# meteofrance/py4cast

Measured on AMD Instinct MI355X. Metric: AR-training samples/sec (512x512x60 grid, 3-step rollout), higher is better.
Workload: dtype bf16; 1 GPU; HalfUNet scaled_ar rollout T=3, grid 512x512x60 (+5 forcings, 4 statics), WeightedLoss(MSE), AdamW, B=2/GPU; global_batch=2, parallelism=dp1, border_size=0, setup_steps=2, accumulate_grad_batches=1, hip_graph=False, deterministic_library_solvers=False, full=False

## Files before the change

### py4cast_amd/csrc/conv_bf16.hip

```cpp
#include <stdlib.h>

#include <type_traits>

#include "kernels.hpp"

namespace p4c {

typedef float f32x16 __attribute__((ext_vector_type(16)));
typedef float f32x4 __attribute__((ext_vector_type(4)));
typedef __bf16 bf16x8 __attribute__((ext_vector_type(8)));
typedef __bf16 bf16x4 __attribute__((ext_vector_type(4)));
typedef short s16x4 __attribute__((ext_vector_type(4)));

constexpr int BTW = 32;

#ifndef P4C_PRIO
#define P4C_PRIO 0
#endif
#ifndef P4C_EXP
#define P4C_EXP 0
#endif

#ifdef P4C_STAMPS
__device__ unsigned long long* g_stamps = nullptr;
// ... 1966 lines not shown
                           in_scale, in_shift, in_relu, out, out_cs, stat_partial, B, H, W);
    if (tag) prof_end(tag, stream);
    P4C_CHECK_LAUNCH("conv_fwd_bf16");
    return P4C_OK;
}

template <typename T, int CI, int KS>
static int launch_conv_wgrad_bf16(const T* in, const float* in_scale, const float* in_shift, int in_relu, const T* dout,
                                  float* partial, int G, int B, int H, int W, int in_cs, int ci_off, int part_cip,
                                  hipStream_t stream) {
    constexpr int HALO = KS / 2;
    constexpr int LH = 8 + 2 * HALO, LW = BTW + 2 * HALO;
    constexpr int ROWA = (CI * 2) % 256 == 64 ? CI * 2 : CI * 2 + 64;
    const size_t smem = (size_t)LH * LW * ROWA + (size_t)8 * BTW * 192;
    auto kern = conv_wgrad_bf16_kernel<T, CI, KS>;
    P4C_TRY(ensure_dyn_smem((const void*)kern, (int)smem));
    const int tag = (CI == 64 && KS == 3 && in_cs == 64) ? P4C_PROF_WGRAD3X3_C64 : 0;
    if (tag) prof_begin(tag, (int64_t)B * H * W, stream);
    hipLaunchKernelGGL(kern, dim3(G), dim3(256), smem, stream, in, in_scale, in_shift, in_relu, dout, partial, B, H, W,
                       in_cs, ci_off, part_cip);
    if (tag) prof_end(tag, stream);
    P4C_CHECK_LAUNCH("conv_wgrad_bf16");
    return P4C_OK;
}

int conv_bf16_stat_slots(int CI, int storage, int B, int H, int W, int ks) {
    if (CI > 96 && ks == 3) return conv_wide_stat_slots(H, W);
    if (conv_bf16_is_rows(storage, CI, ks, 1, 64, B, H, W)) return conv_rows_stat_slots(B, H, W);
    const int tiles = ((H + 3) / 4) * ((W + BTW - 1) / BTW);
    if (CI > 64 && storage != P4C_BF16) return tiles;
    int64_t ntiles = (int64_t)tiles * B;
    const int G = ntiles < num_cus() ? (int)ntiles : num_cus();
    return G * 4;
}

template <typename T>
static int conv_fwd_bf16_t(const T* in, int CI, const void* wp, int ks, const float* in_scale, const float* in_shift,
                           int in_relu, T* out, int out_cs, float* stat_partial, int B, int H, int W, int m_blocks,
                           hipStream_t stream) {
    const __bf16* w = (const __bf16*)wp;
    if (CI > 96 && ks == 3)
        return launch_conv_fwd_bf16_wide<T>(in, CI, w, in_scale, in_shift, in_relu, out, out_cs, stat_partial, B, H, W, m_blocks, stream);
#define P4C_CASE(ci, k, nb)                                                                                          \
    if (CI == ci && ks == k)                                                                                         \
        return launch_conv_fwd_bf16<T, ci, k, nb>(in, w, in_scale, in_shift, in_relu, out, out_cs, stat_partial, B, H, \
                                                  W, m_blocks, stream);
    P4C_CASE(32, 3, 2) P4C_CASE(64, 3, 2) P4C_CASE(96, 3, 1) P4C_CASE(32, 1, 2) P4C_CASE(64, 1, 2) P4C_CASE(96, 1, 1)
#undef P4C_CASE
    return fail(P4C_ERR_UNSUPPORTED, "conv_fwd_bf16: unsupported (CI=%d, ks=%d)", CI, ks);
}

static bool is_tile_ring(int storage, int CI, int ks, int m_blocks, int out_cs, int B, int H, int W) {
    return storage == P4C_BF16 && CI == 64 && ks == 3 && m_blocks == 1 && out_cs % 8 == 0 && B <= ring::MAXB &&
           (int64_t)H * W * out_cs * 2 < (int64_t)1 << 31;
}

bool conv_bf16_is_ring(int storage, int CI, int ks, int m_blocks, int out_cs, int B, int H, int W) {
    return conv_bf16_is_rows(storage, CI, ks, m_blocks, out_cs, B, H, W) || is_tile_ring(storage, CI, ks, m_blocks, out_cs, B, H, W);
}

bool conv_bf16_bwd_stats_ok(int storage, int B, int H, int W) {
    if (conv_bf16_is_rows(storage, 64, 3, 1, 64, B, H, W)) return conv_rows_stat_slots(B, H, W) <= NORM_BWD_MAX_BLOCKS;
    return is_tile_ring(storage, 64, 3, 1, 64, B, H, W) && B <= RING_BWD_STATS_MAXB && 4 * num_cus() <= NORM_BWD_MAX_BLOCKS;
}

int conv_fwd_bf16(const void* in, int storage, int CI, const void* wp, int ks, const float* in_scale,
                  const float* in_shift, int in_relu, void* out, int out_cs, float* stat_partial, int B, int H, int W,
                  int m_blocks, hipStream_t stream, const BatchFin* fin, const RingBwdStats* bst, int* nblk_out, const NormBwdCoef* nb) {
    if (conv_bf16_is_rows(storage, CI, ks, m_blocks, out_cs, B, H, W))
        return launch_conv3x3_bf16_rows(in, wp, ks, in_scale, in_shift, in_relu, out, out_cs, stat_partial, B, H, W, stream, fin, bst,
                                        nblk_out, nb);
    if (nb) return fail(P4C_ERR_INVALID, "conv_fwd_bf16: NormBwdCoef needs the row kernel");
    if (is_tile_ring(storage, CI, ks, m_blocks, out_cs, B, H, W))
        return launch_conv3x3_bf16_ring((const __bf16*)in, (const __bf16*)wp, in_scale, in_shift, in_relu, (__bf16*)out, out_cs,
                                        stat_partial, B, H, W, stream, fin, bst, nblk_out);
    if (fin || bst) return fail(P4C_ERR_INVALID, "conv_fwd_bf16: in-kernel statistics need the ring kernel");
    if (storage == P4C_BF16)
        return conv_fwd_bf16_t<__bf16>((const __bf16*)in, CI, wp, ks, in_scale, in_shift, in_relu, (__bf16*)out, out_cs,
                                       stat_partial, B, H, W, m_blocks, stream);
    return conv_fwd_bf16_t<float>((const float*)in, CI, wp, ks, in_scale, in_shift, in_relu, (float*)out, out_cs, stat_partial,
                                  B, H, W, m_blocks, stream);
}

int wgrad_reduce(const float* partial, int nslots, int ks, int CI_pad, int ci_lo, int ci_hi, int CO, int CI, float* grad,
                 hipStream_t stream);

template <typename T>
static int conv_wgrad_bf16_t(const T* in, int CI, int ks, const float* in_scale, const float* in_shift, int in_relu,
                             const T* dout, float* partial, int G, int B, int H, int W, int CO, int CIreal, float* grad,
                             hipStream_t stream, const NormBwdCoef* nb) {
    if (diag_skip(32)) return P4C_OK;
    if (CI % 32 != 0 || CI <= 0 || CI > 256) return fail(P4C_ERR_UNSUPPORTED, "conv_wgrad_bf16: unsupported CI=%d", CI);
    if (ks != 1 && ks != 3) return fail(P4C_ERR_UNSUPPORTED, "conv_wgrad_bf16: unsupported ks=%d", ks);
    const int tiles = ((H + 7) / 8) * ((W + BTW - 1) / BTW) * B;
    if (tiles < G) G = tiles;
    for (int off = 0; off < CI;) {
        const int chunk = (CI - off >= 64) ? 64 : 32;
        int rc;
        if (std::is_same<T, __bf16>::value && conv_wgrad_rows_ok(P4C_BF16, CI, off, 64, ks, G, B, H, W)) {
            int nslots = 0;
            if (off < CIreal) {
                P4C_TRY(launch_conv3x3_wgrad_bf16_rows(in, in_scale, in_shift, in_relu, dout, partial, G, B, H, W, stream, nb, &nslots, CI, off,
                                                       CIreal, CI));
                if (!diag_skip(8)) P4C_TRY(wgrad_reduce(partial, nslots, 3, CI, off, off + chunk, CO, CIreal, grad, stream));
            }
            off += chunk;
            continue;
        }
        const bool rem_ws = chunk == 32 && ks == 3 && off > 0 && diag_env("P4C_WGWS_REM") != nullptr;
        const bool ws_ok = (chunk == 64 || rem_ws) && (ks == 3 || diag_env("P4C_NO_WGWS_1X1") == nullptr) && std::is_same<T, __bf16>::value &&
                           B <= wgws::MAXB && diag_env("P4C_NO_WGWS") == nullptr;
        if (nb && !ws_ok) return fail(P4C_ERR_INVALID, "conv_wgrad_bf16: NormBwdCoef needs the role-split 3x3 kernel (64-channel chunk, bf16)");
        if (ws_ok)
            rc = launch_conv3x3_wgrad_bf16_ws((const __bf16*)in, in_scale, in_shift, in_relu, (const __bf16*)dout, partial, G, B, H, W,
                                              CI, off, CI, stream, nb, ks);
        else if (chunk == 64 && ks == 3)
            rc = launch_conv_wgrad_bf16<T, 64, 3>(in, in_scale, in_shift, in_relu, dout, partial, G, B, H, W, CI, off, CI, stream);
        else if (chunk == 32 && ks == 3)
            rc = launch_conv_wgrad_bf16<T, 32, 3>(in, in_scale, in_shift, in_relu, dout, partial, G, B, H, W, CI, off, CI, stream);
        else if (chunk == 64)
            rc = launch_conv_wgrad_bf16<T, 64, 1>(in, in_scale, in_shift, in_relu, dout, partial, G, B, H, W, CI, off, CI, stream);
        else
            rc = launch_conv_wgrad_bf16<T, 32, 1>(in, in_scale, in_shift, in_relu, dout, partial, G, B, H, W, CI, off, CI, stream);
        if (rc != P4C_OK) return rc;
        rc = diag_skip(8) ? P4C_OK : wgrad_reduce(partial, G * ((chunk == 64 || ws_ok) ? 1 : 2), ks, CI, off, off + chunk, CO, CIreal, grad, stream);
        if (rc != P4C_OK) return rc;
        off += chunk;
    }
    return P4C_OK;
}

bool conv_wgrad_bf16_takes_nb(int storage, int CI, int ks, int B) {
    if (storage != P4C_BF16 || ks != 3 || B > wgws::MAXB || diag_env("P4C_NO_WGWS")) return false;
    return CI % 64 == 0 || (CI % 64 == 32 && CI > 64 && diag_env("P4C_WGWS_REM") != nullptr);
}

int conv_wgrad_bf16(const void* in, int storage, int CI, int ks, const float* in_scale, const float* in_shift, int in_relu,
                    const void* dout, float* partial, int G, int B, int H, int W, int CO, int CIreal, float* grad,
                    hipStream_t stream, const NormBwdCoef* nb) {
    if (storage == P4C_BF16)
        return conv_wgrad_bf16_t<__bf16>((const __bf16*)in, CI, ks, in_scale, in_shift, in_relu, (const __bf16*)dout, partial, G,
                                         B, H, W, CO, CIreal, grad, stream, nb);
    if (nb) return fail(P4C_ERR_INVALID, "conv_wgrad_bf16: NormBwdCoef needs bf16 storage");
    return conv_wgrad_bf16_t<float>((const float*)in, CI, ks, in_scale, in_shift, in_relu, (const float*)dout, partial, G, B, H,
                                    W, CO, CIreal, grad, stream, nullptr);
}

int conv_wgrad_bf16_compact(const void* in, int in_cs, int ks, const void* dout, int dout_cs, float* partial, int G, int B, int H, int W,
                            int CO, int CIreal, float* grad, hipStream_t stream) {
    if (in_cs <= 0 || dout_cs <= 0 || in_cs > 64 || dout_cs > 64 || in_cs % 8 || dout_cs % 8 || (ks != 1 && ks != 3) || B > wgws::MAXB)
        return fail(P4C_ERR_UNSUPPORTED, "conv_wgrad_bf16_compact: unsupported shape (%d / %d channels, ks %d, B %d)", in_cs, dout_cs, ks, B);
    P4C_TRY(launch_conv3x3_wgrad_bf16_ws((const __bf16*)in, nullptr, nullptr, 0, (const __bf16*)dout, partial, G, B, H, W, in_cs, 0, 64, stream,
                                         nullptr, ks, dout_cs));
    const int tiles = ((H + 3) / 4) * ((W + BTW - 1) / BTW) * B;
    return wgrad_reduce(partial, tiles < G ? tiles : G, ks, 64, 0, 64, CO, CIreal, grad, stream);
}

#ifdef P4C_STAMPS
}
extern "C" int p4c_debug_set_stamps(void* p) {
    return hipMemcpyToSymbol(HIP_SYMBOL(p4c::g_stamps), &p, sizeof(p)) == hipSuccess ? 0 : -1;
}
namespace p4c {
#endif

int prep_weights_bf16(const float* w, int CO, int CI, int ks, int transpose_flip, int M_pad, int K_pad, void* out,
                      hipStream_t stream) {
    const int total = M_pad * K_pad * ks * ks;
    hipLaunchKernelGGL(prep_weights_bf16_kernel, dim3((total + 255) / 256), dim3(256), 0, stream, w, CO, CI, ks * ks,
                       transpose_flip, M_pad, K_pad, (__bf16*)out);
    P4C_CHECK_LAUNCH("prep_weights_bf16");
    return P4C_OK;
}

__global__ void __launch_bounds__(256) prep_weights_batch_kernel(PrepBatch pb) {
    if (blockIdx.x == 0 && blockIdx.y == 0 && (int)threadIdx.x < pb.n_zero) pb.zero_words[threadIdx.x] = 0u;
    const PrepJob& jb = pb.job[blockIdx.y];
    const int total = jb.M_pad * jb.K_pad * jb.ntaps;
    const int kv = pb.bf16 ? 8 : 4;
    const int ksteps = jb.K_pad / (2 * kv);
    for (int i = blockIdx.x * 256 + threadIdx.x; i < total; i += gridDim.x * 256) {
// ... 35 lines not shown
```

### py4cast_amd/csrc/conv_f32.hip

```cpp
#include "kernels.hpp"

namespace p4c {

typedef float f32x16 __attribute__((ext_vector_type(16)));
typedef float f32x4 __attribute__((ext_vector_type(4)));

constexpr int TW = 32;

__global__ void prep_weights_kernel(const float* __restrict__ w, int CO, int CI, int ntaps, int transpose_flip,
                                    int M_pad, int K_pad, float* __restrict__ out) {
    const int total = M_pad * K_pad * ntaps;
    for (int i = blockIdx.x * blockDim.x + threadIdx.x; i < total; i += gridDim.x * blockDim.x) {
        int t = i;
        const int s = t & 3; t >>= 2;
        const int m_l = t & 63; t >>= 6;
        const int h = t & 1; t >>= 1;
        const int q = t % (K_pad / 8); t /= (K_pad / 8);
        const int tap = t % ntaps;
        const int mb = t / ntaps;
        const int k = 8 * q + 4 * h + s, m = 64 * mb + m_l;
        float v = 0.0f;
        if (!transpose_flip) {
            if (m < CO && k < CI) v = w[((int64_t)m * CI + k) * ntaps + tap];
        } else {
// ... 185 lines not shown
    constexpr int KSPLIT = 4 / UNITS;
    constexpr int KSTEPS = TH * TW / 2 / KSPLIT;
    extern __shared__ __attribute__((aligned(16))) float lds[];
    float* lin = lds;
    float* ldo = lds + LH * LW * CIS;

    const int lane = threadIdx.x & 63, wv = threadIdx.x >> 6;
    const int r = lane & 31, h = lane >> 5;
    const int unit = wv % UNITS, ksl = wv / UNITS;
    const int cit = unit >> 1, cot = unit & 1;
    const int tiles_x = (W + TW - 1) / TW, tiles_y = (H + TH - 1) / TH;
    const int ntiles = tiles_x * tiles_y * B;
    const float* inb = in + ci_off;
    const float* scb = in_scale ? in_scale + ci_off : nullptr;
    const float* shb = in_shift ? in_shift + ci_off : nullptr;

    f32x16 acc[NTAPS];
#pragma unroll
    for (int t = 0; t < NTAPS; ++t)
#pragma unroll
        for (int i = 0; i < 16; ++i) acc[t][i] = 0.f;

    TileRegs<CI, LH, LW> tr;
    f32x4 dreg[TH * TW * 16 / 256];
    auto load_tile = [&](int tile) {
        const int tx = tile % tiles_x;
        const int rest = tile / tiles_x;
        const int ty = rest % tiles_y, b = rest / tiles_y;
        tile_load<CI, LH, LW, HALO>(tr, inb, b, ty * TH, tx * TW, H, W, in_cs);
#pragma unroll
        for (int it = 0; it < TH * TW * 16 / 256; ++it) {
            const int idx = threadIdx.x + it * 256;
            const int pix = idx >> 4, c4 = idx & 15;
            const int gy = ty * TH + (pix >> 5), gx = tx * TW + (pix & 31);
            f32x4 v = {0.f, 0.f, 0.f, 0.f};
            if (gy < H && gx < W) v = *reinterpret_cast<const f32x4*>(dout + (((int64_t)b * H + gy) * W + gx) * 64 + 4 * c4);
            dreg[it] = v;
        }
    };
    auto store_tile = [&](int tile) {
        const int tx = tile % tiles_x;
        const int rest = tile / tiles_x;
        const int ty = rest % tiles_y, b = rest / tiles_y;
        tile_store<CI, LH, LW, HALO>(tr, scb, shb, in_relu, lin, b, ty * TH, tx * TW, H, W, in_cs);
#pragma unroll
        for (int it = 0; it < TH * TW * 16 / 256; ++it) {
            const int idx = threadIdx.x + it * 256;
            *reinterpret_cast<f32x4*>(ldo + (idx >> 4) * DS + 4 * (idx & 15)) = dreg[it];
        }
    };

    int tile = blockIdx.x;
    if (tile < ntiles) load_tile(tile);
    for (; tile < ntiles; tile += gridDim.x) {
        __syncthreads();
        store_tile(tile);
        __syncthreads();
        if (tile + (int)gridDim.x < ntiles) load_tile(tile + gridDim.x);
#pragma unroll 2
        for (int kp = 0; kp < KSTEPS; ++kp) {
            const int p = 2 * (ksl * KSTEPS + kp) + h;
            const int row = p >> 5, col = p & 31;
            const float bv = ldo[p * DS + cot * 32 + r];
            const float* ain = lin + (row * LW + col) * CIS + cit * 32 + r;
#pragma unroll
            for (int t = 0; t < NTAPS; ++t) {
                const int ky = t / KS, kx = t - ky * KS;
                acc[t] = __builtin_amdgcn_mfma_f32_32x32x2f32(ain[(ky * LW + kx) * CIS], bv, acc[t], 0, 0, 0);
            }
        }
    }
    float* pbase = partial + ((int64_t)blockIdx.x * KSPLIT + ksl) * NTAPS * part_cip * 64;
#pragma unroll
    for (int t = 0; t < NTAPS; ++t)
#pragma unroll
        for (int i = 0; i < 16; ++i) {
            const int ci = ci_off + cit * 32 + (i & 3) + 8 * (i >> 2) + 4 * h;
            pbase[((int64_t)t * part_cip + ci) * 64 + cot * 32 + r] = acc[t][i];
        }
}

template <int QL>
__device__ __forceinline__ void wgrad_reduce_block(const float* __restrict__ partial, int nslots, int ntaps, int CI_pad, int ci_lo,
                                                   int ci_hi, int CO, int CI, float* __restrict__ grad, int block) {
    constexpr int NS = 256 / QL, NCO = 4 * QL, NG = 64 / NCO;
    __shared__ float red[NS][NCO];
    const int nci = ci_hi - ci_lo;
    const int cg = block % NG, rest = block / NG;
    const int tap = rest / nci, ci = ci_lo + (rest - tap * nci);
    const int q = threadIdx.x % QL, sl = threadIdx.x / QL;
    const int64_t stride = (int64_t)ntaps * CI_pad * 64;
    const float* p = partial + ((int64_t)tap * CI_pad + ci) * 64 + cg * NCO + 4 * q;
    f32x4 s = {0.f, 0.f, 0.f, 0.f};
#pragma unroll 8
    for (int g = sl; g < nslots; g += NS) s += *reinterpret_cast<const f32x4*>(p + g * stride);
#pragma unroll
    for (int j = 0; j < 4; ++j) red[sl][4 * q + j] = s[j];
    __syncthreads();
    if (threadIdx.x < NCO) {
        const int co = cg * NCO + threadIdx.x;
        float t = 0.f;
#pragma unroll
        for (int k = 0; k < NS; ++k) t += red[k][threadIdx.x];
        if (co < CO && ci < CI) grad[((int64_t)co * CI + ci) * ntaps + tap] += t;
    }
}

template <int QL>
__global__ void __launch_bounds__(256) wgrad_reduce_kernel(const float* __restrict__ partial, int nslots, int ntaps, int CI_pad,
                                                           int ci_lo, int ci_hi, int CO, int CI, float* __restrict__ grad) {
    wgrad_reduce_block<QL>(partial, nslots, ntaps, CI_pad, ci_lo, ci_hi, CO, CI, grad, blockIdx.x);
}

struct WgradBatchArgs {
    WgradReduceJob job[WGRAD_BATCH_MAX];
    int first[WGRAD_BATCH_MAX + 1];
    int n;
};
__global__ void __launch_bounds__(256) wgrad_reduce_batch_kernel(WgradBatchArgs a) {
    int j = 0;
    while (j + 1 < a.n && (int)blockIdx.x >= a.first[j + 1]) ++j;
    const WgradReduceJob& J = a.job[j];
    wgrad_reduce_block<16>(J.partial, J.nslots, J.ntaps, J.CI_pad, J.ci_lo, J.ci_hi, J.CO, J.CI, J.grad, (int)blockIdx.x - a.first[j]);
}

template <int KS>
__global__ void __launch_bounds__(256)
    conv_fwd_f32_wide_kernel(const float* __restrict__ in, int CI, const float* __restrict__ wp, const float* __restrict__ in_scale,
                             const float* __restrict__ in_shift, int in_relu, float* __restrict__ out, int out_cs,
                             float* __restrict__ stat_partial, int H, int W) {
    constexpr int CC = 32;
    constexpr int TH = 4;
    constexpr int HALO = KS / 2;
    constexpr int LH = TH + 2 * HALO, LW = TW + 2 * HALO;
    constexpr int CIS = CC + 4;
    constexpr int NTAPS = KS * KS;
    constexpr int NQ = CC / 8;
    extern __shared__ __attribute__((aligned(16))) float lds[];

    const int NC = CI / CC, NQT = CI / 8;
    const int tiles_y = (H + TH - 1) / TH;
    const int b = blockIdx.y / tiles_y, ty = blockIdx.y - b * tiles_y;
    const int y0 = ty * TH, x0 = blockIdx.x * TW;
    const int mb = blockIdx.z;
    const int lane = threadIdx.x & 63, wv = threadIdx.x >> 6;
    const int r = lane & 31, h = lane >> 5;

    f32x16 acc[2];
#pragma unroll
    for (int ct = 0; ct < 2; ++ct)
#pragma unroll
        for (int i = 0; i < 16; ++i) acc[ct][i] = 0.f;

    const float* wbase = wp + (int64_t)mb * NTAPS * CI * 64 + (h * 64 + r) * 4;
    TileRegs<CC, LH, LW> tr;
    tile_load<CC, LH, LW, HALO>(tr, in, b, y0, x0, H, W, CI);
#pragma unroll 1
    for (int c = 0; c < NC; ++c) {
        __syncthreads();
        tile_store<CC, LH, LW, HALO>(tr, in_scale ? in_scale + c * CC : nullptr, in_shift ? in_shift + c * CC : nullptr, in_relu, lds, b,
                                     y0, x0, H, W, CI);
        __syncthreads();
        if (c + 1 < NC) tile_load<CC, LH, LW, HALO>(tr, in + (c + 1) * CC, b, y0, x0, H, W, CI);
        f32x4 a0 = *reinterpret_cast<const f32x4*>(wbase + (int64_t)(4 * c) * 512);
        f32x4 a1 = *reinterpret_cast<const f32x4*>(wbase + (int64_t)(4 * c) * 512 + 128);
#pragma unroll 1
        for (int tap = 0; tap < NTAPS; ++tap) {
            const int ky = tap / KS, kx = tap - ky * KS;
            const float* lt = lds + ((wv + ky) * LW + (r + kx)) * CIS + 4 * h;
#pragma unroll
            for (int q = 0; q < NQ; ++q) {
                const int tn = q + 1 < NQ ? tap : (tap + 1 < NTAPS ? tap + 1 : tap);
                const int qn = q + 1 < NQ ? q + 1 : 0;
                const int64_t jn = (int64_t)tn * NQT + 4 * c + qn;
                const f32x4 n0 = *reinterpret_cast<const f32x4*>(wbase + jn * 512);
                const f32x4 n1 = *reinterpret_cast<const f32x4*>(wbase + jn * 512 + 128);
                const f32x4 bb = *reinterpret_cast<const f32x4*>(lt + 8 * q);
#pragma unroll
                for (int s = 0; s < 4; ++s) {
                    acc[0] = __builtin_amdgcn_mfma_f32_32x32x2f32(a0[s], bb[s], acc[0], 0, 0, 0);
                    acc[1] = __builtin_amdgcn_mfma_f32_32x32x2f32(a1[s], bb[s], acc[1], 0, 0, 0);
                }
                a0 = n0;
                a1 = n1;
            }
        }
    }

    const int gx = x0 + r;
    const int gy = y0 + wv;
    const bool valid = (gy < H) && (gx < W);
    __syncthreads();
    float* tw = lds + wv * (64 * 33);
    float* orow = out + (((int64_t)b * H + gy) * W + gx) * out_cs + mb * 64 + 4 * h;
#pragma unroll
    for (int ct = 0; ct < 2; ++ct) {
#pragma unroll
        for (int g = 0; g < 4; ++g) {
            const f32x4 v = {acc[ct][4 * g], acc[ct][4 * g + 1], acc[ct][4 * g + 2], acc[ct][4 * g + 3]};
            if (valid) *reinterpret_cast<f32x4*>(orow + ct * 32 + 8 * g) = v;
            if (stat_partial) {
#pragma unroll
                for (int j = 0; j < 4; ++j) tw[(ct * 32 + 8 * g + 4 * h + j) * 33 + r] = valid ? v[j] : 0.f;
            }
        }
    }
// ... 30 lines not shown
    if (smem < stat_smem) smem = stat_smem;
    auto kern = conv_fwd_f32_wide_kernel<3>;
    P4C_TRY(ensure_dyn_smem((const void*)kern, (int)smem));
    const int tiles_x = (W + TW - 1) / TW, tiles_y = (H + 3) / 4;
    hipLaunchKernelGGL(kern, dim3(tiles_x, tiles_y * B, m_blocks), dim3(256), smem, stream, in, CI, wp, in_scale, in_shift, in_relu, out,
                       out_cs, stat_partial, H, W);
    P4C_CHECK_LAUNCH("conv_fwd_f32_wide");
    return P4C_OK;
}

template <int CI, int KS, int TH>
static int launch_conv_fwd(const float* in, const float* wp, const float* in_scale, const float* in_shift, int in_relu,
                           const float* bias, float* out, int out_cs, float* stat_partial, int B, int H, int W,
                           int m_blocks, hipStream_t stream) {
    constexpr int HALO = KS / 2;
    constexpr int LH = TH + 2 * HALO, LW = TW + 2 * HALO;
    size_t smem = (size_t)LH * LW * (CI + 4) * sizeof(float);
    const size_t stat_smem = (4 * 64 * 33 + 4 * 2 * 64) * sizeof(float);
    if (smem < stat_smem) smem = stat_smem;
    auto kern = conv_fwd_f32_kernel<CI, KS, TH>;
    P4C_TRY(ensure_dyn_smem((const void*)kern, (int)smem));
    const int tiles_x = (W + TW - 1) / TW, tiles_y = (H + TH - 1) / TH;
    const int tag = (CI == 64 && KS == 3 && m_blocks == 1) ? P4C_PROF_CONV3X3_C64 : 0;
    if (tag) prof_begin(tag, (int64_t)B * H * W, stream);
    hipLaunchKernelGGL(kern, dim3(tiles_x, tiles_y * B, m_blocks), dim3(256), smem, stream, in, wp, in_scale, in_shift,
                       in_relu, bias, out, out_cs, stat_partial, H, W);
    if (tag) prof_end(tag, stream);
    P4C_CHECK_LAUNCH("conv_fwd_f32");
    return P4C_OK;
}

template <int CI, int KS>
static int launch_conv_wgrad(const float* in, const float* in_scale, const float* in_shift, int in_relu,
                             const float* dout, float* partial, int G, int B, int H, int W, int in_cs, int ci_off,
                             int part_cip, hipStream_t stream) {
    constexpr int HALO = KS / 2;
    constexpr int LH = 4 + 2 * HALO, LW = TW + 2 * HALO;
    const size_t smem = ((size_t)LH * LW * (CI + 4) + (size_t)4 * TW * 68) * sizeof(float);
    auto kern = conv_wgrad_f32_kernel<CI, KS>;
    P4C_TRY(ensure_dyn_smem((const void*)kern, (int)smem));
    const int tag = (CI == 64 && KS == 3 && in_cs == 64) ? P4C_PROF_WGRAD3X3_C64 : 0;
    if (tag) prof_begin(tag, (int64_t)B * H * W, stream);
    hipLaunchKernelGGL(kern, dim3(G), dim3(256), smem, stream, in, in_scale, in_shift, in_relu, dout, partial, B, H, W,
                       in_cs, ci_off, part_cip);
    if (tag) prof_end(tag, stream);
    P4C_CHECK_LAUNCH("conv_wgrad_f32");
    return P4C_OK;
}

int conv_fwd_f32(const float* in, int CI, const float* wp, int ks, const float* in_scale, const float* in_shift,
                 int in_relu, const float* bias, float* out, int out_cs, float* stat_partial, int B, int H, int W,
                 int m_blocks, hipStream_t stream) {
    if (CI > 96 && ks == 3 && !bias)
        return launch_conv_fwd_f32_wide(in, CI, wp, in_scale, in_shift, in_relu, out, out_cs, stat_partial, B, H, W, m_blocks, stream);
#define P4C_CASE(ci, k)                                                                                              \
    if (CI == ci && ks == k)                                                                                         \
        return launch_conv_fwd<ci, k, 4>(in, wp, in_scale, in_shift, in_relu, bias, out, out_cs, stat_partial, B, H, \
                                         W, m_blocks, stream);
    P4C_CASE(32, 3) P4C_CASE(64, 3) P4C_CASE(96, 3) P4C_CASE(32, 1) P4C_CASE(64, 1) P4C_CASE(96, 1)
#undef P4C_CASE
    return fail(P4C_ERR_UNSUPPORTED, "conv_fwd_f32: unsupported (CI=%d, ks=%d): CI must be 32/64/96, ks 1/3", CI, ks);
}

static thread_local WgradCollect* g_wgrad_collect = nullptr;
void wgrad_collect_into(WgradCollect* c) { g_wgrad_collect = c; }

int wgrad_reduce_batch(const WgradCollect& c, hipStream_t stream) {
    if (c.n == 0) return P4C_OK;
    WgradBatchArgs a;
    a.n = c.n;
    int blocks = 0;
    for (int j = 0; j < c.n; ++j) {
        a.job[j] = c.job[j];
        a.first[j] = blocks;
        blocks += c.job[j].ntaps * (c.job[j].ci_hi - c.job[j].ci_lo);
    }
    a.first[c.n] = blocks;
    hipLaunchKernelGGL(wgrad_reduce_batch_kernel, dim3(blocks), dim3(256), 0, stream, a);
    P4C_CHECK_LAUNCH("wgrad_reduce_batch");
    return P4C_OK;
}

int wgrad_reduce(const float* partial, int nslots, int ks, int CI_pad, int ci_lo, int ci_hi, int CO, int CI, float* grad,
                        hipStream_t stream) {
    if (ci_hi > CI) ci_hi = CI;
    if (ci_hi <= ci_lo) return P4C_OK;
    if (WgradCollect* c = g_wgrad_collect) {
        if (c->n == WGRAD_BATCH_MAX) return fail(P4C_ERR_INVALID, "wgrad_reduce: more than %d deferred reductions in one batch", WGRAD_BATCH_MAX);
        c->job[c->n++] = WgradReduceJob{partial, grad, nslots, ks * ks, CI_pad, ci_lo, ci_hi, CO, CI};
        return P4C_OK;
    }
    const int pairs = ks * ks * (ci_hi - ci_lo);
    if (pairs < 256 && nslots >= 64)
        hipLaunchKernelGGL(wgrad_reduce_kernel<4>, dim3(pairs * 4), dim3(256), 0, stream, partial, nslots, ks * ks, CI_pad, ci_lo,
                           ci_hi, CO, CI, grad);
    else
        hipLaunchKernelGGL(wgrad_reduce_kernel<16>, dim3(pairs), dim3(256), 0, stream, partial, nslots, ks * ks, CI_pad, ci_lo, ci_hi,
                           CO, CI, grad);
    P4C_CHECK_LAUNCH("wgrad_reduce");
    return P4C_OK;
}

int conv_wgrad_f32(const float* in, int CI, int ks, const float* in_scale, const float* in_shift, int in_relu,
                   const float* dout, float* partial, int G, int B, int H, int W, int CO, int CIreal, float* grad,
                   hipStream_t stream) {
    if (CI % 32 != 0 || CI <= 0 || CI > 256) return fail(P4C_ERR_UNSUPPORTED, "conv_wgrad_f32: unsupported CI=%d", CI);
    if (ks != 1 && ks != 3) return fail(P4C_ERR_UNSUPPORTED, "conv_wgrad_f32: unsupported ks=%d", ks);
    for (int off = 0; off < CI;) {
        const int chunk = (CI - off >= 64) ? 64 : 32;
        int rc;
        if (chunk == 64 && ks == 3)
            rc = launch_conv_wgrad<64, 3>(in, in_scale, in_shift, in_relu, dout, partial, G, B, H, W, CI, off, CI, stream);
        else if (chunk == 32 && ks == 3)
            rc = launch_conv_wgrad<32, 3>(in, in_scale, in_shift, in_relu, dout, partial, G, B, H, W, CI, off, CI, stream);
        else if (chunk == 64)
            rc = launch_conv_wgrad<64, 1>(in, in_scale, in_shift, in_relu, dout, partial, G, B, H, W, CI, off, CI, stream);
        else
            rc = launch_conv_wgrad<32, 1>(in, in_scale, in_shift, in_relu, dout, partial, G, B, H, W, CI, off, CI, stream);
        if (rc != P4C_OK) return rc;
        const int nslots = G * (chunk == 64 ? 1 : 2);
        rc = wgrad_reduce(partial, nslots, ks, CI, off, off + chunk, CO, CIreal, grad, stream);
        if (rc != P4C_OK) return rc;
        off += chunk;
    }
    return P4C_OK;
}

int prep_weights(const float* w, int CO, int CI, int ks, int transpose_flip, int M_pad, int K_pad, float* out,
                 hipStream_t stream) {
    const int total = M_pad * K_pad * ks * ks;
    hipLaunchKernelGGL(prep_weights_kernel, dim3((total + 255) / 256), dim3(256), 0, stream, w, CO, CI, ks * ks,
                       transpose_flip, M_pad, K_pad, out);
    P4C_CHECK_LAUNCH("prep_weights");
    return P4C_OK;
}

}
```

### py4cast_amd/csrc/conv_thin.hip

```cpp
#include "kernels.hpp"

namespace p4c {
namespace {

typedef float f32x16 __attribute__((ext_vector_type(16)));
typedef float f32x4 __attribute__((ext_vector_type(4)));
typedef __bf16 bf16x8 __attribute__((ext_vector_type(8)));
typedef unsigned int u32x4 __attribute__((ext_vector_type(4)));

constexpr int OOB = 0x7fffffff;
constexpr int SP = 68;
constexpr int WIMG_BYTES = 2 * 5 * 64 * 16;

struct ThinArgs {
    const __bf16* x;
    const float* w;
    __bf16* y;
    float* stat_partial;
    int x_cs, c0, nc, cin;
    int H, W, nblk;
};

__device__ __forceinline__ float bf_lo(unsigned int w) { return __builtin_bit_cast(float, w << 16); }
__device__ __forceinline__ float bf_hi(unsigned int w) { return __builtin_bit_cast(float, w & 0xffff0000u); }
__device__ __forceinline__ unsigned int pack2(float lo, float hi) {
    typedef float f32x2 __attribute__((ext_vector_type(2)));
    typedef __bf16 bf16x2 __attribute__((ext_vector_type(2)));
    const f32x2 v = {lo, hi};
    return __builtin_bit_cast(unsigned int, __builtin_convertvector(v, bf16x2));
}

__global__ void __launch_bounds__(256) first_conv_tail_kernel(ThinArgs a) {
    __shared__ __attribute__((aligned(16))) char smem[WIMG_BYTES + 4 * 32 * SP * 4];
    __bf16* wimg = reinterpret_cast<__bf16*>(smem);
    const int tid = threadIdx.x, lane = tid & 63, wv = tid >> 6, r = lane & 31, h = lane >> 5;
    float* tile = reinterpret_cast<float*>(smem + WIMG_BYTES) + wv * 32 * SP;
    for (int idx = tid; idx < 2 * 5 * 64; idx += 256) {
        const int l = idx & 63, ts = idx >> 6;
        const int s = ts % 5, ct = ts / 5;
        const int co = 32 * ct + (l & 31), tap = 2 * s + (l >> 5);
        bf16x8 o;
#pragma unroll
        for (int j = 0; j < 8; ++j) o[j] = (__bf16)((tap < 9 && j < a.nc) ? a.w[((int64_t)co * a.cin + a.c0 + j) * 9 + tap] : 0.f);
        *reinterpret_cast<bf16x8*>(wimg + idx * 8) = o;
    }
    __syncthreads();
    bf16x8 A[2][5];
#pragma unroll
    for (int ct = 0; ct < 2; ++ct)
#pragma unroll
        for (int s = 0; s < 5; ++s) A[ct][s] = *reinterpret_cast<const bf16x8*>(wimg + ((ct * 5 + s) * 64 + lane) * 8);

    const int b = blockIdx.y, H = a.H, W = a.W;
    const int64_t npix = (int64_t)H * W;
    const __amdgpu_buffer_rsrc_t rs_x = __builtin_amdgcn_make_buffer_rsrc(const_cast<__bf16*>(a.x + (int64_t)b * npix * a.x_cs), 0,
                                                                        (int)(npix * a.x_cs * 2), 0x00020000);
    __bf16* yb = a.y + (int64_t)b * npix * 64;
    const int ngroups = (int)(npix / 32);
    const int wid = blockIdx.x * 4 + wv, nwaves = a.nblk * 4;
    const int prow = lane >> 3, c8 = lane & 7;
    float a1[8], a2[8];
#pragma unroll
    for (int q = 0; q < 8; ++q) a1[q] = a2[q] = 0.f;

    auto load_group = [&](int g, bf16x8 (&bop)[5], u32x4 (&yq)[4]) __attribute__((always_inline)) {
        const bool live = g < ngroups;
        const int p0 = live ? g * 32 : 0, yy = p0 / W, x0 = p0 - yy * W;
#pragma unroll
        for (int s = 0; s < 5; ++s) {
            const int tap = 2 * s + h, dy = tap / 3 - 1, dx = tap - (tap / 3) * 3 - 1;
            const int sy = yy + dy, sx = x0 + r + dx;
            const bool ok = live && tap < 9 && (unsigned)sy < (unsigned)H && (unsigned)sx < (unsigned)W;
            const u32x4 v = __builtin_amdgcn_raw_buffer_load_b128(rs_x, ok ? ((sy * W + sx) * a.x_cs + a.c0) * 2 : OOB, 0, 0);
            bop[s] = __builtin_bit_cast(bf16x8, v);
        }
#pragma unroll
        for (int it = 0; it < 4; ++it) yq[it] = *reinterpret_cast<const u32x4*>(yb + ((int64_t)p0 + 8 * it + prow) * 64 + 8 * c8);
    };
    bf16x8 Bop[5], Bnx[5];
    u32x4 yv[4], ynx[4];
    load_group(wid, Bop, yv);
    for (int g = wid; g < ngroups; g += nwaves) {
        const int p0 = g * 32;
        load_group(g + nwaves, Bnx, ynx);
        f32x16 acc[2];
#pragma unroll
        for (int ct = 0; ct < 2; ++ct) {
#pragma unroll
            for (int i = 0; i < 16; ++i) acc[ct][i] = 0.f;
#pragma unroll
            for (int s = 0; s < 5; ++s) acc[ct] = __builtin_amdgcn_mfma_f32_32x32x16_bf16(A[ct][s], Bop[s], acc[ct], 0, 0, 0);
        }
#pragma unroll
        for (int ct = 0; ct < 2; ++ct)
#pragma unroll
            for (int q = 0; q < 4; ++q)
                *reinterpret_cast<f32x4*>(tile + r * SP + 32 * ct + 8 * q + 4 * h) = f32x4{acc[ct][4 * q], acc[ct][4 * q + 1], acc[ct][4 * q + 2], acc[ct][4 * q + 3]};
        __builtin_amdgcn_wave_barrier();
        asm volatile("" ::: "memory");
#pragma unroll
        for (int it = 0; it < 4; ++it) {
            const int px = 8 * it + prow;
            const f32x4 t0 = *reinterpret_cast<const f32x4*>(tile + px * SP + 8 * c8), t1 = *reinterpret_cast<const f32x4*>(tile + px * SP + 8 * c8 + 4);
            const float t[8] = {t0[0], t0[1], t0[2], t0[3], t1[0], t1[1], t1[2], t1[3]};
            u32x4 o;
#pragma unroll
            for (int k = 0; k < 4; ++k) {
                o[k] = pack2(bf_lo(yv[it][k]) + t[2 * k], bf_hi(yv[it][k]) + t[2 * k + 1]);
                const float lo = bf_lo(o[k]), hi = bf_hi(o[k]);
                a1[2 * k] += lo; a2[2 * k] = __builtin_fmaf(lo, lo, a2[2 * k]);
                a1[2 * k + 1] += hi; a2[2 * k + 1] = __builtin_fmaf(hi, hi, a2[2 * k + 1]);
            }
            *reinterpret_cast<u32x4*>(yb + ((int64_t)p0 + px) * 64 + 8 * c8) = o;
        }
        __builtin_amdgcn_wave_barrier();
        asm volatile("" ::: "memory");
#pragma unroll
        for (int s = 0; s < 5; ++s) Bop[s] = Bnx[s];
#pragma unroll
        for (int it = 0; it < 4; ++it) yv[it] = ynx[it];
    }
    if (a.stat_partial) {
        float* dst = a.stat_partial + ((int64_t)b * nwaves + wid) * 128;
#pragma unroll
        for (int q = 0; q < 8; ++q) {
            float u = a1[q], v = a2[q];
            u += __shfl_xor(u, 8); v += __shfl_xor(v, 8);
            u += __shfl_xor(u, 16); v += __shfl_xor(v, 16);
            u += __shfl_xor(u, 32); v += __shfl_xor(v, 32);
            if (lane < 8) { dst[8 * c8 + q] = u; dst[64 + 8 * c8 + q] = v; }
        }
    }
}

int tail_blocks(int B, int H, int W) {
    const int64_t groups = (int64_t)H * W / 32;
    int64_t n = (groups + 3) / 4;
    if (n > 256) n = 256;
    const int64_t cap = 2 * (int64_t)num_cus() / (B > 0 ? B : 1);
    if (n > cap && cap >= 1) n = cap;
    return n < 1 ? 1 : (int)n;
}

}

bool first_conv_split_ok(int compute, int storage, int cin, int cin_pad, int B, int H, int W) {
    const char* e = diag_env("P4C_FIRST_CONV_SPLIT");
    if (e && e[0] == '0') return false;
    return compute == P4C_BF16 && storage == P4C_BF16 && cin_pad == 96 && cin > 64 && cin <= 72 && W % 32 == 0 &&
           conv_bf16_is_rows(storage, 64, 3, 1, 64, B, H, W) && (int64_t)H * W * 192 < ((int64_t)1 << 31);
}

int first_conv_tail_slots(int B, int H, int W) { return tail_blocks(B, H, W) * 4; }

int launch_first_conv_tail(const void* x, int x_cs, int cin, const float* w, void* y, float* stat_partial, int B, int H, int W, hipStream_t stream) {
    ThinArgs a{(const __bf16*)x, w, (__bf16*)y, stat_partial, x_cs, 64, cin - 64, cin, H, W, tail_blocks(B, H, W)};
    hipLaunchKernelGGL(first_conv_tail_kernel, dim3(a.nblk, B), dim3(256), 0, stream, a);
    P4C_CHECK_LAUNCH("first_conv_tail");
    return P4C_OK;
}

}

extern "C" int p4c_first_conv_tail_slots(int B, int H, int W) { return p4c::first_conv_tail_slots(B, H, W); }
extern "C" int p4c_first_conv_tail(const void* x, int x_cs, int cin, const float* w, void* y, float* stat_partial, int B, int H, int W,
                                   p4c_stream_t stream) {
    P4C_CHECK_ARG(x && w && y, "p4c_first_conv_tail: NULL pointer");
    P4C_CHECK_ARG(cin > 64 && cin <= 72 && x_cs >= 72 && x_cs % 8 == 0 && W % 32 == 0 && B > 0 && H > 0,
                  "p4c_first_conv_tail: 65..72 input channels on pixels of >= 72 channels (multiple of 8), W a multiple of 32");
    return p4c::launch_first_conv_tail(x, x_cs, cin, w, y, stat_partial, B, H, W, p4c::as_stream(stream));
}
```

### py4cast_amd/csrc/kernels.hpp

```cpp
#pragma once
#include "common.hpp"

namespace p4c {

int prep_weights(const float* w, int CO, int CI, int ks, int transpose_flip, int M_pad, int K_pad, float* out,
                 hipStream_t stream);
int conv_fwd_f32(const float* in, int CI, const float* wp, int ks, const float* in_scale, const float* in_shift,
                 int in_relu, const float* bias, float* out, int out_cs, float* stat_partial, int B, int H, int W,
                 int m_blocks, hipStream_t stream);
int conv_wgrad_f32(const float* in, int CI, int ks, const float* in_scale, const float* in_shift, int in_relu,
                   const float* dout, float* partial, int G, int B, int H, int W, int CO, int CIreal, float* grad,
                   hipStream_t stream);
static inline int64_t wgrad_partial_floats(int CI_pad, int ks, int G) { return (int64_t)2 * G * ks * ks * CI_pad * 64; }

int wgrad_reduce(const float* partial, int nslots, int ks, int CI_pad, int ci_lo, int ci_hi, int CO, int CI, float* grad,
                 hipStream_t stream);
struct WgradReduceJob {
    const float* partial;
    float* grad;
    int nslots, ntaps, CI_pad, ci_lo, ci_hi, CO, CI;
};
constexpr int WGRAD_BATCH_MAX = 24;
struct WgradCollect {
    WgradReduceJob job[WGRAD_BATCH_MAX];
    int n = 0;
};
void wgrad_collect_into(WgradCollect* c);
int wgrad_reduce_batch(const WgradCollect& c, hipStream_t stream);

int prep_weights_bf16(const float* w, int CO, int CI, int ks, int transpose_flip, int M_pad, int K_pad, void* out,
                      hipStream_t stream);
struct PrepJob {
    const float* w;
    void* out;
    int CO, CI, ntaps, transpose_flip, M_pad, K_pad;
};
struct PrepBatch {
    PrepJob job[32];
    int n;
    int bf16;
    unsigned int* zero_words;
    int n_zero;
};

struct BatchFin {
    float* slots;
    unsigned int* ticket;
    const float* gamma;
    const float* beta;
    float* running_mean;
    float* running_var;
    float* scale;
    float* shift;
    float* mean;
    float* rstd;
    double count;
    float eps, momentum;
    int B;
};
struct BwdFin {
    unsigned int* ticket;
    const float* gamma;
    float* dgamma;
    float* dbeta;
    float* k1;
    float* k2;
    float count;
    int B, training;
};
int bwd_fin_max_slots();
int prep_weights_batch(const PrepBatch& pb, hipStream_t stream);
int conv_bf16_stat_slots(int CI, int storage, int B, int H, int W, int ks = 3);
struct RingBwdStats {
    const void* y;
    const float* scale;
    const float* shift;
    const float* mean;
    const float* rstd;
};
constexpr int RING_BWD_STATS_MAXB = 21;
struct NormBwdCoef {
    const void* y;
    const float* gamma;
    const float* scale;
    const float* shift;
    const float* rstd;
    const float* mean;
    const float* k1;
    const float* k2;
};
int conv_fwd_bf16(const void* in, int storage, int CI, const void* wp, int ks, const float* in_scale,
                  const float* in_shift, int in_relu, void* out, int out_cs, float* stat_partial, int B, int H, int W,
                  int m_blocks, hipStream_t stream, const BatchFin* fin = nullptr, const RingBwdStats* bst = nullptr,
                  int* nblk_out = nullptr, const NormBwdCoef* nb = nullptr);
bool conv_bf16_norm_bwd_fused_ok(int storage, int CI, int B, int H, int W);
bool conv_bf16_is_ring(int storage, int CI, int ks, int m_blocks, int out_cs, int B, int H, int W);
bool conv_bf16_bwd_stats_ok(int storage, int B, int H, int W);

bool conv_bf16_is_rows(int storage, int CI, int ks, int m_blocks, int out_cs, int B, int H, int W);
void conv_rows_geometry(int B, int H, int W, int* nstrips, int* nseg);
int conv_rows_stat_slots(int B, int H, int W);
int launch_conv3x3_bf16_rows(const void* in, const void* wp, int ks, const float* in_scale, const float* in_shift, int in_relu,
                             void* out, int out_cs, float* stat_partial, int B, int H, int W, hipStream_t stream, const BatchFin* fin,
                             const RingBwdStats* bst, int* nblk_out, const NormBwdCoef* nb = nullptr);
int conv_wgrad_bf16(const void* in, int storage, int CI, int ks, const float* in_scale, const float* in_shift, int in_relu,
                    const void* dout, float* partial, int G, int B, int H, int W, int CO, int CIreal, float* grad,
                    hipStream_t stream, const NormBwdCoef* nb = nullptr);
bool conv_wgrad_rows_ok(int storage, int in_cs, int ci_off, int dout_cs, int ks, int G, int B, int H, int W);
int launch_conv3x3_wgrad_bf16_rows(const void* x, const float* x_scale, const float* x_shift, int x_relu, const void* dout, float* partial,
                                   int G, int B, int H, int W, hipStream_t stream, const NormBwdCoef* nb, int* nslots_out, int in_cs = 64,
                                   int ci_off = 0, int ci_real = 64, int part_cip = 64);
bool out_conv_bwd_ok(int storage, int B, int64_t N);
int out_conv_bwd_slots(int B, int64_t N);
int launch_out_conv_bwd(const void* dy, const void* wp_dgrad, const void* y, const float* scale, const float* shift, const float* mean,
                        const float* rstd, void* dA, float* stat_partial, float* wpartial, int B, int64_t N, hipStream_t stream,
                        int* nblk_out);
bool conv_wgrad_bf16_takes_nb(int storage, int CI, int ks, int B);
bool conv_rows_compact_ok(int storage, int in_cs, int out_cs, int ks, int B, int H, int W);
int launch_conv_bf16_rows_compact(const void* in, int in_cs, const void* wp, int ks, void* out, int out_cs, int B, int H, int W,
                                  hipStream_t stream);
int conv_wgrad_bf16_compact(const void* in, int in_cs, int ks, const void* dout, int dout_cs, float* partial, int G, int B, int H, int W,
                            int CO, int CIreal, float* grad, hipStream_t stream);

bool first_conv_split_ok(int compute, int storage, int cin, int cin_pad, int B, int H, int W);
int first_conv_tail_slots(int B, int H, int W);
int launch_first_conv_tail(const void* x, int x_cs, int cin, const float* w, void* y, float* stat_partial, int B, int H, int W, hipStream_t stream);
int launch_conv_bf16_rows_wide_pixels(const void* in, int pixel_channels, const void* wp, void* out, int B, int H, int W, hipStream_t stream);

int norm_finalize(const float* partial, int tiles_per_sample, int B, int64_t hw, int mode, int groups, const float* gamma,
                  const float* beta, float eps, float momentum, float* running_mean, float* running_var, float* scale,
                  float* shift, float* mean, float* rstd, hipStream_t stream);
int norm_eval(int B, const float* gamma, const float* beta, float eps, const float* running_mean,
              const float* running_var, float* scale, float* shift, float* mean, float* rstd, hipStream_t stream);
int norm_bwd_blocks(int64_t hw);
int norm_bwd(int storage, const void* dA, const void* y, const float* scale, const float* shift, const float* mean,
             const float* rstd, const float* gamma, int relu, int B, int64_t hw, int mode, int groups, int training,
             float* partial, float* k1, float* k2, float* dgamma, float* dbeta, void* dY, hipStream_t stream, int pre_nblk = 0,
             unsigned int* fin_ticket = nullptr, bool pre_finalized = false);
constexpr int NORM_BWD_MAX_BLOCKS = 1024;
int pool_fwd(int storage, const void* y, const float* scale, const float* shift, int B, int H, int W, void* P,
             hipStream_t stream);
int upsum_fwd(int storage, const void* const* y, const float* const* scale, const float* const* shift, int B, int H, int W,
              void* S, hipStream_t stream);
int up_bwd_x4(int storage, const void* dS, int B, int H, int W, void* const* tx, hipStream_t stream);
bool up_bwd_x4_mfma_ok(int B, int H, int W);
int launch_up_bwd_x4_mfma(const void* dS, int64_t rows, int W, void* const* tx, hipStream_t stream);
int enc_out_bwd(int storage, const void* Tx, int Hfull, int s, const void* dS, const void* dP, const void* y,
                const float* scale, const float* shift, int B, int Hk, int Wk, void* dA, hipStream_t stream,
                const float* mean = nullptr, const float* rstd = nullptr, float* partial = nullptr, int* nblk_out = nullptr,
                const BwdFin* fin = nullptr, bool* finalized_out = nullptr);

constexpr int GRAD_JOB_MLP = 0, GRAD_JOB_PROJ = 1;
struct GradReduceJob {
    const float* partial;
    int slots, n, kind, K;
    float* p[6];
    int ld[3];
    int k_real, o_real;
};
int grad_reduce_submit(const GradReduceJob& job, hipStream_t stream, int defer);
int tn_reduce_flush(hipStream_t stream);
int tn_reduce_pending();
void tn_reduce_drop();

constexpr int CONV_TH = 4;
constexpr int CONV_TW = 32;
static inline int conv_tiles_per_sample(int H, int W) { return ((H + CONV_TH - 1) / CONV_TH) * ((W + CONV_TW - 1) / CONV_TW); }

}
```

Baseline: 445.2 samples/s.

## Add thin-channel wgrad kernel for the 64..72 input-channel tail of first conv

Adds a dedicated 3x3 weight-gradient kernel for the 8-channel remainder (channels 64-72 of a 96-padded input) instead of running the generic 32-channel chunk path over mostly padded channels. The kernel streams rows through LDS rings, uses transposed LDS reads into bf16 MFMA, and writes a compact 8-channel partial slab. wgrad_reduce gains a ci_base offset so it can index that compact partial. This avoids computing and reducing gradients for padding channels, but it adds a new specialized kernel and places its scratch region after the main partial buffer, which may overrun that buffer if it was not sized for it.

```diff
diff --git a/py4cast_amd/csrc/conv_bf16.hip b/py4cast_amd/csrc/conv_bf16.hip
--- a/py4cast_amd/csrc/conv_bf16.hip
+++ b/py4cast_amd/csrc/conv_bf16.hip
@@ -2072,9 +2072,6 @@
                                   B, H, W, m_blocks, stream);
 }
 
-int wgrad_reduce(const float* partial, int nslots, int ks, int CI_pad, int ci_lo, int ci_hi, int CO, int CI, float* grad,
-                 hipStream_t stream);
-
 template <typename T>
 static int conv_wgrad_bf16_t(const T* in, int CI, int ks, const float* in_scale, const float* in_shift, int in_relu,
                              const T* dout, float* partial, int G, int B, int H, int W, int CO, int CIreal, float* grad,
@@ -2087,6 +2084,15 @@
     for (int off = 0; off < CI;) {
         const int chunk = (CI - off >= 64) ? 64 : 32;
         int rc;
+        if (std::is_same<T, __bf16>::value && off == 64 && !in_scale && !in_relu && !nb &&
+            conv_wgrad_thin_ok(P4C_BF16, CI, CIreal, 64, ks, B, H, W)) {
+            int nslots = 0;
+            float* thin = partial + (int64_t)G * 9 * CI * 64;
+            P4C_TRY(launch_conv3x3_wgrad_thin_bf16(in, CI, dout, thin, G, B, H, W, stream, &nslots));
+            if (!diag_skip(8)) P4C_TRY(wgrad_reduce(thin, nslots, 3, 8, 64, 72, CO, CIreal, grad, stream, 64));
+            off += chunk;
+            continue;
+        }
         if (std::is_same<T, __bf16>::value && conv_wgrad_rows_ok(P4C_BF16, CI, off, 64, ks, G, B, H, W)) {
             int nslots = 0;
             if (off < CIreal) {
diff --git a/py4cast_amd/csrc/conv_f32.hip b/py4cast_amd/csrc/conv_f32.hip
--- a/py4cast_amd/csrc/conv_f32.hip
+++ b/py4cast_amd/csrc/conv_f32.hip
@@ -291,7 +291,7 @@
 
 template <int QL>
 __device__ __forceinline__ void wgrad_reduce_block(const float* __restrict__ partial, int nslots, int ntaps, int CI_pad, int ci_lo,
-                                                   int ci_hi, int CO, int CI, float* __restrict__ grad, int block) {
+                                                   int ci_hi, int CO, int CI, float* __restrict__ grad, int block, int ci_base) {
     constexpr int NS = 256 / QL, NCO = 4 * QL, NG = 64 / NCO;
     __shared__ float red[NS][NCO];
     const int nci = ci_hi - ci_lo;
@@ -299,7 +299,7 @@
     const int tap = rest / nci, ci = ci_lo + (rest - tap * nci);
     const int q = threadIdx.x % QL, sl = threadIdx.x / QL;
     const int64_t stride = (int64_t)ntaps * CI_pad * 64;
-    const float* p = partial + ((int64_t)tap * CI_pad + ci) * 64 + cg * NCO + 4 * q;
+    const float* p = partial + ((int64_t)tap * CI_pad + (ci - ci_base)) * 64 + cg * NCO + 4 * q;
     f32x4 s = {0.f, 0.f, 0.f, 0.f};
 #pragma unroll 8
     for (int g = sl; g < nslots; g += NS) s += *reinterpret_cast<const f32x4*>(p + g * stride);
@@ -317,8 +317,8 @@
 
 template <int QL>
 __global__ void __launch_bounds__(256) wgrad_reduce_kernel(const float* __restrict__ partial, int nslots, int ntaps, int CI_pad,
-                                                           int ci_lo, int ci_hi, int CO, int CI, float* __restrict__ grad) {
-    wgrad_reduce_block<QL>(partial, nslots, ntaps, CI_pad, ci_lo, ci_hi, CO, CI, grad, blockIdx.x);
+                                                           int ci_lo, int ci_hi, int CO, int CI, float* __restrict__ grad, int ci_base) {
+    wgrad_reduce_block<QL>(partial, nslots, ntaps, CI_pad, ci_lo, ci_hi, CO, CI, grad, blockIdx.x, ci_base);
 }
 
 struct WgradBatchArgs {
@@ -330,7 +330,7 @@
     int j = 0;
     while (j + 1 < a.n && (int)blockIdx.x >= a.first[j + 1]) ++j;
     const WgradReduceJob& J = a.job[j];
-    wgrad_reduce_block<16>(J.partial, J.nslots, J.ntaps, J.CI_pad, J.ci_lo, J.ci_hi, J.CO, J.CI, J.grad, (int)blockIdx.x - a.first[j]);
+    wgrad_reduce_block<16>(J.partial, J.nslots, J.ntaps, J.CI_pad, J.ci_lo, J.ci_hi, J.CO, J.CI, J.grad, (int)blockIdx.x - a.first[j], J.ci_base);
 }
 
 template <int KS>
@@ -527,21 +527,21 @@
 }
 
 int wgrad_reduce(const float* partial, int nslots, int ks, int CI_pad, int ci_lo, int ci_hi, int CO, int CI, float* grad,
-                        hipStream_t stream) {
+                        hipStream_t stream, int ci_base) {
     if (ci_hi > CI) ci_hi = CI;
     if (ci_hi <= ci_lo) return P4C_OK;
     if (WgradCollect* c = g_wgrad_collect) {
         if (c->n == WGRAD_BATCH_MAX) return fail(P4C_ERR_INVALID, "wgrad_reduce: more than %d deferred reductions in one batch", WGRAD_BATCH_MAX);
-        c->job[c->n++] = WgradReduceJob{partial, grad, nslots, ks * ks, CI_pad, ci_lo, ci_hi, CO, CI};
+        c->job[c->n++] = WgradReduceJob{partial, grad, nslots, ks * ks, CI_pad, ci_lo, ci_hi, CO, CI, ci_base};
         return P4C_OK;
     }
     const int pairs = ks * ks * (ci_hi - ci_lo);
     if (pairs < 256 && nslots >= 64)
         hipLaunchKernelGGL(wgrad_reduce_kernel<4>, dim3(pairs * 4), dim3(256), 0, stream, partial, nslots, ks * ks, CI_pad, ci_lo,
-                           ci_hi, CO, CI, grad);
+                           ci_hi, CO, CI, grad, ci_base);
     else
         hipLaunchKernelGGL(wgrad_reduce_kernel<16>, dim3(pairs), dim3(256), 0, stream, partial, nslots, ks * ks, CI_pad, ci_lo, ci_hi,
-                           CO, CI, grad);
+                           CO, CI, grad, ci_base);
     P4C_CHECK_LAUNCH("wgrad_reduce");
     return P4C_OK;
 }
diff --git a/py4cast_amd/csrc/conv_thin.hip b/py4cast_amd/csrc/conv_thin.hip
--- a/py4cast_amd/csrc/conv_thin.hip
+++ b/py4cast_amd/csrc/conv_thin.hip
@@ -1,3 +1,5 @@
+#include <stdlib.h>
+
 #include "kernels.hpp"
 
 namespace p4c {
@@ -160,6 +162,199 @@
     return P4C_OK;
 }
 
+namespace {
+namespace wt {
+constexpr int SW = 64, LW = SW + 2;
+constexpr int RPI = 2;
+constexpr int NRX = 8, NRD = 2 * RPI;
+constexpr int XROW = LW * 16, DROW = SW * 128;
+constexpr int XRING = NRX * XROW, DRING = NRD * DROW;
+constexpr int SLAB = 9 * 8 * 64;
+__device__ __forceinline__ int slot_off(int col, int c8) { return col * 128 + ((((c8 >> 2) ^ (col >> 1)) & 1) << 6) + ((c8 & 3) << 4); }
+}
+
+typedef short s16x4 __attribute__((ext_vector_type(4)));
+__device__ __forceinline__ s16x4 tr_read(const char* p) {
+    return __builtin_amdgcn_ds_read_tr16_b64_v4i16((s16x4 __attribute__((address_space(3)))*)(p));
+}
+
+struct WgThinArgs {
+    const __bf16* x;
+    const __bf16* dout;
+    float* partial;
+    int H, W, in_cs, c0, nseg, nstrips, nitems;
+};
+
+__global__ void __launch_bounds__(256) conv3x3_wgrad_thin_bf16_kernel(WgThinArgs a) {
+    using namespace wt;
+    __shared__ __attribute__((aligned(16))) char smem[XRING + DRING];
+    char* xring = smem;
+    char* dring = smem + XRING;
+    const int tid = threadIdx.x, lane = tid & 63, wv = tid >> 6;
+    const int cot = wv & 1, kh = wv >> 1;
+    const int h = lane >> 5, r = lane & 31;
+    const int tq = (lane & 15) >> 2, tp = lane & 3, tg = (lane >> 4) & 1;
+    const int H = a.H, W = a.W, xpb = a.in_cs * 2;
+
+    int ky[3], xo[3];
+#pragma unroll
+    for (int t = 0; t < 3; ++t) {
+        int tap = 4 * t + 2 * tg + (tp >> 1);
+        tap = tap > 8 ? 8 : tap;
+        ky[t] = tap / 3;
+        xo[t] = (32 * kh + 8 * h + tq + (tap - 3 * ky[t])) * 16 + (tp & 1) * 8;
+    }
+    const int doff = (32 * kh + 8 * h + tq) * 128 + (((cot ^ (tq >> 1)) & 1) << 6) + (tg * 16 + tp * 4) * 2;
+    f32x16 acc[3];
+#pragma unroll
+    for (int t = 0; t < 3; ++t)
+#pragma unroll
+        for (int i = 0; i < 16; ++i) acc[t][i] = 0.f;
+
+    const int c8 = tid & 7;
+    int gd[4], ld[4];
+#pragma unroll
+    for (int j = 0; j < 4; ++j) {
+        const int px = (tid + j * 256) >> 3, row = px >> 6, col = px & 63;
+        gd[j] = (row * W + col) * 128 + 16 * c8;
+        ld[j] = row * DROW + slot_off(col, c8);
+    }
+    const bool xlive = tid < 2 * LW;
+    const int xr = tid >= LW ? 1 : 0, xc = tid - xr * LW;
+
+    for (int item = blockIdx.x; item < a.nitems; item += gridDim.x) {
+        const int seg = item % a.nseg, rest = item / a.nseg;
+        const int strip = rest % a.nstrips, b = rest / a.nstrips;
+        const int rows_lo = H / a.nseg, rows_rem = H % a.nseg;
+        const int y0 = seg * rows_lo + (seg < rows_rem ? seg : rows_rem);
+        const int R = rows_lo + (seg < rows_rem ? 1 : 0);
+        const int x0 = strip * SW;
+        const int K = (R + RPI - 1) / RPI;
+        const __amdgpu_buffer_rsrc_t rs_x = __builtin_amdgcn_make_buffer_rsrc(
+            const_cast<__bf16*>(a.x + (int64_t)b * H * W * a.in_cs + a.c0), 0, (int)(((int64_t)H * W * a.in_cs - a.c0) * 2), 0x00020000);
+        const __amdgpu_buffer_rsrc_t rs_d = __builtin_amdgcn_make_buffer_rsrc(
+            const_cast<__bf16*>(a.dout + (int64_t)b * H * W * 64), 0, (int)((int64_t)H * W * 128), 0x00020000);
+        auto loadx = [&](int m0) __attribute__((always_inline)) {
+            const int m = m0 + xr, gy = y0 - 1 + m, gx = x0 - 1 + xc;
+            const bool ok = xlive & (m <= R + 1) & ((unsigned)gy < (unsigned)H) & ((unsigned)gx < (unsigned)W);
+            return __builtin_amdgcn_raw_buffer_load_b128(rs_x, ok ? (gy * W + gx) * xpb : OOB, 0, 0);
+        };
+        auto storex = [&](u32x4 v, int m0) __attribute__((always_inline)) {
+            if (xlive) *reinterpret_cast<u32x4*>(xring + ((m0 + xr) & (NRX - 1)) * XROW + xc * 16) = v;
+        };
+        auto loadd = [&](u32x4 (&d)[4], int k) __attribute__((always_inline)) {
+            int ndr = R - RPI * k;
+            ndr = ndr > RPI ? RPI : (ndr < 0 ? 0 : ndr);
+            const int sd = ((y0 + RPI * k) * W + x0) * 128;
+#pragma unroll
+            for (int j = 0; j < 4; ++j) d[j] = __builtin_amdgcn_raw_buffer_load_b128(rs_d, (tid + j * 256 < ndr * 512) ? gd[j] : OOB, ndr ? sd : 0, 0);
+        };
+        auto stored = [&](const u32x4 (&d)[4], int k) __attribute__((always_inline)) {
+            int ndr = R - RPI * k;
+            ndr = ndr > RPI ? RPI : (ndr < 0 ? 0 : ndr);
+            char* dst = dring + ((RPI * k) & (NRD - 1)) * DROW;
+#pragma unroll
+            for (int j = 0; j < 4; ++j)
+                if (tid + j * 256 < ndr * 512) *reinterpret_cast<u32x4*>(dst + ld[j]) = d[j];
+        };
+        u32x4 xa, da[4];
+        __syncthreads();
+        xa = loadx(0);
+        storex(xa, 0);
+        xa = loadx(2);
+        loadd(da, 0);
+        storex(xa, 2);
+        stored(da, 0);
+        xa = loadx(4);
+        loadd(da, 1);
+        __syncthreads();
+        for (int k = 0; k < K; ++k) {
+#pragma unroll
+            for (int rr = 0; rr < RPI; ++rr) {
+                const int n = RPI * k + rr;
+                if (n < R) {
+                    const char* dr = dring + (n & (NRD - 1)) * DROW + doff;
+                    int xb[3];
+#pragma unroll
+                    for (int t = 0; t < 3; ++t) xb[t] = ((n + ky[t]) & (NRX - 1)) * XROW + xo[t];
+#pragma unroll
+                    for (int s = 0; s < 2; ++s) {
+                        union { s16x4 q[2]; bf16x8 v; } ub;
+                        ub.q[0] = tr_read(dr + s * 2048);
+                        ub.q[1] = tr_read(dr + s * 2048 + 512);
+#pragma unroll
+                        for (int t = 0; t < 3; ++t) {
+                            union { s16x4 q[2]; bf16x8 v; } ua;
+                            ua.q[0] = tr_read(xring + xb[t] + s * 256);
+                            ua.q[1] = tr_read(xring + xb[t] + s * 256 + 64);
+                            acc[t] = __builtin_amdgcn_mfma_f32_32x32x16_bf16(ua.v, ub.v, acc[t], 0, 0, 0);
+                        }
+                    }
+                }
+            }
+            storex(xa, 2 * k + 4);
+            stored(da, k + 1);
+            xa = loadx(2 * k + 6);
+            loadd(da, k + 2);
+            __syncthreads();
+        }
+    }
+    float* red = reinterpret_cast<float*>(dring);
+    __syncthreads();
+    if (kh == 1) {
+#pragma unroll
+        for (int t = 0; t < 3; ++t)
+#pragma unroll
+            for (int i = 0; i < 16; ++i) red[((cot * 48 + t * 16 + i) << 6) + lane] = acc[t][i];
+    }
+    __syncthreads();
+    if (kh == 0) {
+        float* pbase = a.partial + (int64_t)blockIdx.x * SLAB;
+#pragma unroll
+        for (int t = 0; t < 3; ++t)
+#pragma unroll
+            for (int i = 0; i < 16; ++i) {
+                const int tap = 4 * t + (i >> 2), c = (i & 3) + 4 * h;
+                if (tap < 9) pbase[(tap * 8 + c) * 64 + cot * 32 + r] = acc[t][i] + red[((cot * 48 + t * 16 + i) << 6) + lane];
+            }
+    }
+}
+
+}
+
+bool conv_wgrad_thin_ok(int storage, int in_cs, int ci_real, int dout_cs, int ks, int B, int H, int W) {
+    const char* e = diag_env("P4C_WGRAD_THIN");
+    if (e && e[0] == '0') return false;
+    const char* r = diag_env("P4C_NO_WGRAD_ROWS");
+    if (r && r[0] == '1') return false;
+    return storage == P4C_BF16 && in_cs == 96 && ci_real > 64 && ci_real <= 72 && dout_cs == 64 && ks == 3 && W % wt::SW == 0 && B > 0 &&
+           H > 0 && (int64_t)H * W * in_cs * 2 < (int64_t)1 << 31;
+}
+
+int conv_wgrad_thin_slots(int G, int B, int H, int W, int* nseg_out) {
+    const int nstrips = W / wt::SW;
+    int g = 2 * G;
+    if (const char* e = diag_env("P4C_WGRAD_THIN_G")) { const int v = atoi(e); if (v > 0) g = v; }
+    if (g > 12 * G) g = 12 * G;
+    int nseg = g / (B * nstrips);
+    nseg = nseg > H ? H : (nseg < 1 ? 1 : nseg);
+    const int nitems = B * nstrips * nseg;
+    if (nseg_out) *nseg_out = nseg;
+    return g < nitems ? g : nitems;
+}
+
+int launch_conv3x3_wgrad_thin_bf16(const void* x, int in_cs, const void* dout, float* partial, int G, int B, int H, int W, hipStream_t stream,
+                                   int* nslots_out) {
+    int nseg = 1;
+    const int nwg = conv_wgrad_thin_slots(G, B, H, W, &nseg);
+    const int nstrips = W / wt::SW;
+    const WgThinArgs a{(const __bf16*)x, (const __bf16*)dout, partial, H, W, in_cs, 64, nseg, nstrips, B * nstrips * nseg};
+    hipLaunchKernelGGL(conv3x3_wgrad_thin_bf16_kernel, dim3(nwg), dim3(256), 0, stream, a);
+    P4C_CHECK_LAUNCH("conv3x3_wgrad_thin_bf16");
+    *nslots_out = nwg;
+    return P4C_OK;
+}
+
 }
 
 extern "C" int p4c_first_conv_tail_slots(int B, int H, int W) { return p4c::first_conv_tail_slots(B, H, W); }
diff --git a/py4cast_amd/csrc/kernels.hpp b/py4cast_amd/csrc/kernels.hpp
--- a/py4cast_amd/csrc/kernels.hpp
+++ b/py4cast_amd/csrc/kernels.hpp
@@ -14,11 +14,12 @@
 static inline int64_t wgrad_partial_floats(int CI_pad, int ks, int G) { return (int64_t)2 * G * ks * ks * CI_pad * 64; }
 
 int wgrad_reduce(const float* partial, int nslots, int ks, int CI_pad, int ci_lo, int ci_hi, int CO, int CI, float* grad,
-                 hipStream_t stream);
+                 hipStream_t stream, int ci_base = 0);
 struct WgradReduceJob {
     const float* partial;
     float* grad;
     int nslots, ntaps, CI_pad, ci_lo, ci_hi, CO, CI;
+    int ci_base = 0;
 };
 constexpr int WGRAD_BATCH_MAX = 24;
 struct WgradCollect {
@@ -125,6 +126,10 @@
 bool first_conv_split_ok(int compute, int storage, int cin, int cin_pad, int B, int H, int W);
 int first_conv_tail_slots(int B, int H, int W);
 int launch_first_conv_tail(const void* x, int x_cs, int cin, const float* w, void* y, float* stat_partial, int B, int H, int W, hipStream_t stream);
+bool conv_wgrad_thin_ok(int storage, int in_cs, int ci_real, int dout_cs, int ks, int B, int H, int W);
+int conv_wgrad_thin_slots(int G, int B, int H, int W, int* nseg_out = nullptr);
+int launch_conv3x3_wgrad_thin_bf16(const void* x, int in_cs, const void* dout, float* partial, int G, int B, int H, int W, hipStream_t stream,
+                                   int* nslots_out);
 int launch_conv_bf16_rows_wide_pixels(const void* in, int pixel_channels, const void* wp, void* out, int B, int H, int W, hipStream_t stream);
 
 int norm_finalize(const float* partial, int tiles_per_sample, int B, int64_t hw, int mode, int groups, const float* gamma,
```

Measured after the change: 450.5 samples/s (median of 6 runs). 1.2% higher.
